# nizepart/Research-and-Development-of-Kubernetes-Operator-for-Machine-Learning-Pipelines

Hardware: AMD Instinct MI355X
Metric: served_tokens_per_sec (higher is better)
Workload: dtype bf16

## Files before the change

research-and-development-of-kubernetes-operator-for-machine-learning-pipelines_amd/ops/__init__.py:

```python
from __future__ import annotations

import math
import os
from pathlib import Path

import torch

from . import reference as ref

_LIB = Path(__file__).resolve().parent / "_C.so"
_loaded = False


class StaleExtension(RuntimeError):
    pass


def load(build_if_missing: bool = True) -> bool:
    global _loaded
    if _loaded:
        return True
    from .build import source_hash

    want = source_hash()
# ... 143 lines not shown


def paged_attention(q, k_cache, v_cache, meta, out: torch.Tensor | None = None,
                    k_scale: torch.Tensor | None = None, v_scale: torch.Tensor | None = None):
    fp8 = _fp8_scales(k_cache, k_scale, v_scale)
    if not q.is_cuda:
        return ref.paged_attention(q, k_cache, v_cache, meta, k_scale, v_scale)
    _need_gpu()
    out = torch.empty_like(q) if out is None else out
    scale = 1.0 / math.sqrt(q.shape[-1])
    window = getattr(meta, "window", 0)
    if fp8:
        pts = getattr(meta, "ptile_seq", None)
        if window or (pts is not None and pts.numel()):
            raise NotImplementedError("fp8 KV cache: no sliding-window and no flash-prefill kernel "
                                      "(build the metadata with flash_min_q = 1 << 30)")
        if meta.tile_seq.numel():
            sem = getattr(meta, "part_sem", None)
            torch.ops.mlop.paged_attention_fp8(out, meta.part_o, meta.part_ml, _no_sem(q.device) if sem is None else sem,
                                               q, k_cache, v_cache, k_scale, v_scale, meta.block_tables,
                                               meta.tile_seq, meta.tile_q0, meta.q_start, meta.q_len, meta.ctx_len,
                                               scale, meta.part_tokens, meta.nparts)
        return out
    if meta.tile_seq.numel():
        sem = getattr(meta, "part_sem", None)
        if sem is None:
            sem = _no_sem(q.device)
        torch.ops.mlop.paged_attention(out, meta.part_o, meta.part_ml, sem, q, k_cache, v_cache,
                                       meta.block_tables, meta.tile_seq, meta.tile_q0, meta.q_start,
                                       meta.q_len, meta.ctx_len, scale, meta.part_tokens, meta.nparts,
                                       window)
    pts = getattr(meta, "ptile_seq", None)
    if pts is not None and pts.numel():
        torch.ops.mlop.flash_prefill(out, q, k_cache, v_cache, meta.block_tables, pts, meta.ptile_q0,
                                     meta.q_start, meta.q_len, meta.ctx_len, scale, window)
    return out


EPI_NONE, EPI_SILU_MUL = 0, 1


def gemm(x: torch.Tensor, w: torch.Tensor, out: torch.Tensor | None = None, epi: int = EPI_NONE):
    N = w.shape[0]
    out_n = N if epi == EPI_NONE else N // 2
    if not x.is_cuda:
        y = torch.nn.functional.linear(x, w) if x.dtype != torch.bfloat16 else \
            torch.nn.functional.linear(x.float(), w.float()).to(x.dtype)
        if epi == EPI_SILU_MUL:
            y = ref.silu_mul(deinterleave_cols(y))
        if out is not None:
            out.copy_(y.view_as(out))
            return out
        return y
    _need_gpu()
    lead = x.shape[:-1]
# ... 646 lines not shown
```

research-and-development-of-kubernetes-operator-for-machine-learning-pipelines_amd/ops/csrc/attention.hip:

```cpp
#include <type_traits>
#include <algorithm>

#include "common.h"
#include "launch.h"

namespace mlop {

__device__ __forceinline__ float fast_exp2(float x) { return __builtin_amdgcn_exp2f(x); }

constexpr int kD = 128;
constexpr int kBS = 16;
constexpr float kNegBig = -1.0e30f;

__device__ __forceinline__ int vswz(int t) { return ((t & 3) << 2) | ((t >> 2) & 3); }
typedef short v4s16 __attribute__((ext_vector_type(4)));
typedef __attribute__((address_space(3))) v4s16 lds_v4s16;

__device__ __forceinline__ uint32_t vt_base(int lane) {
  const int g4 = lane >> 4, q = (lane >> 2) & 3, p = lane & 3;
  const int row = 8 * g4 + q, sw = vswz(row & 15);
  return 256u * row + 16u * ((p >> 1) ^ (sw & 1)) + 8u * (p & 1) + 32u * (sw >> 1);
}
__device__ __forceinline__ bf16x8 vt_frag(uint32_t b, int d) {
  const uint32_t a0 = b ^ (32u * d), a1 = (a0 ^ 16u) + 1024u;
  const v4s16 lo = __builtin_amdgcn_ds_read_tr16_b64_v4i16((lds_v4s16*)(uintptr_t)a0);
  const v4s16 hi = __builtin_amdgcn_ds_read_tr16_b64_v4i16((lds_v4s16*)(uintptr_t)a1);
  bf16x8 f;
#pragma unroll
  for (int e = 0; e < 4; ++e) {
    f[e] = lo[e];
    f[4 + e] = hi[e];
  }
  return f;
}

__device__ __forceinline__ int wid_of(unsigned t) { return __builtin_amdgcn_readfirstlane((int)(t >> 6)); }

__device__ __forceinline__ int window_kv_lo(int p0, int window) { return max(0, p0 - window + 1) & ~31; }


struct KvBf16 {
  const uint16_t* kc;
  const uint16_t* vc;
  static constexpr bool kScaled = false;
  struct Pair {};
  static __device__ __forceinline__ int q_dim(int kk, int g4) { return kk * 32 + g4 * 8; }
  template <int NT>
  __device__ __forceinline__ void load_k(Pair&, int pgA, int pgB, size_t page_stride, int kvh, int lane,
                                         bf16x8 (&ka)[4], bf16x8 (&kb)[4]) const {
    const int r = lane & 15, g4 = lane >> 4;
    const uint16_t* kA = kc + pgA * page_stride + (size_t)kvh * kBS * kD;
    const uint16_t* kB = kc + pgB * page_stride + (size_t)kvh * kBS * kD;
    const uint16_t* kR = (r >> 3 ? kB : kA) + (8 * ((r >> 2) & 1) + (r & 3)) * kD;
#pragma unroll
    for (int kk = 0; kk < 4; ++kk) {
      if constexpr ((NT & 1) != 0) {
        ka[kk] = __builtin_nontemporal_load(reinterpret_cast<const bf16x8*>(kR + kk * 32 + g4 * 8));
        kb[kk] = __builtin_nontemporal_load(reinterpret_cast<const bf16x8*>(kR + 4 * kD + kk * 32 + g4 * 8));
      } else {
        ka[kk] = *reinterpret_cast<const bf16x8*>(kR + kk * 32 + g4 * 8);
        kb[kk] = *reinterpret_cast<const bf16x8*>(kR + 4 * kD + kk * 32 + g4 * 8);
      }
    }
  }
  template <int NT>
  __device__ __forceinline__ void issue_v(Pair&, int pgA, int pgB, size_t page_stride, int kvh, int lane,
                                          uint32_t vimg) const {
    const int r = lane & 15, g4 = lane >> 4;
    asm volatile("s_waitcnt lgkmcnt(0)" ::: "memory");
    const uint16_t* vA = vc + pgA * page_stride + (size_t)kvh * kBS * kD;
    const uint16_t* vB = vc + pgB * page_stride + (size_t)kvh * kBS * kD;
#pragma unroll
    for (int i = 0; i < 8; ++i) {
      const int trow = (4 * i + g4) & 15;
      const uint16_t* src = (i < 4 ? vA : vB) + trow * kD + ((r ^ vswz(trow)) << 3);
      __builtin_amdgcn_global_load_lds((const void*)src, (lds_void_t*)(uintptr_t)(vimg + 1024u * i), 16, 0,
                                       (NT & 1) ? 2  : 0);
    }
  }
  __device__ __forceinline__ void v_ready(const Pair&, int, uint32_t) const {
    asm volatile("s_waitcnt vmcnt(0)" ::: "memory");
  }
  __device__ __forceinline__ void v_read_done() const {}
};

typedef __attribute__((address_space(3))) u32x4 lds_u32x4;

__device__ __forceinline__ bf16x8 cvt8(uint32_t w0, uint32_t w1) {
  const auto f0 = __builtin_amdgcn_cvt_pk_f32_fp8((int)w0, false);
  const auto f1 = __builtin_amdgcn_cvt_pk_f32_fp8((int)w0, true);
  const auto f2 = __builtin_amdgcn_cvt_pk_f32_fp8((int)w1, false);
  const auto f3 = __builtin_amdgcn_cvt_pk_f32_fp8((int)w1, true);
  u32x4 o;
  o[0] = __builtin_amdgcn_perm(__float_as_uint(f0[1]), __float_as_uint(f0[0]), 0x07060302u);
  o[1] = __builtin_amdgcn_perm(__float_as_uint(f1[1]), __float_as_uint(f1[0]), 0x07060302u);
  o[2] = __builtin_amdgcn_perm(__float_as_uint(f2[1]), __float_as_uint(f2[0]), 0x07060302u);
  o[3] = __builtin_amdgcn_perm(__float_as_uint(f3[1]), __float_as_uint(f3[0]), 0x07060302u);
  return __builtin_bit_cast(bf16x8, o);
// ... 1 lines not shown

__device__ __forceinline__ float scale_of(uint32_t w, int i) {
  return __uint_as_float(((w >> (8 * i)) & 0xffu) << 23);
}

template <bool NT>
__device__ __forceinline__ u32x4 load16(const uint8_t* p) {
  if constexpr (NT) return __builtin_nontemporal_load(reinterpret_cast<const u32x4*>(p));
  else return *reinterpret_cast<const u32x4*>(p);
}

struct KvFp8 {
  const uint8_t* kc;
  const uint8_t* vc;
  const uint8_t* ksc;
  const uint8_t* vsc;
  int srow_stride;
  static constexpr bool kScaled = true;
  struct Pair {
    u32x2 ksw, vsw;
    u32x4 vr[4];
  };
  static __device__ __forceinline__ int q_dim(int kk, int g4) { return 64 * (kk >> 1) + 16 * g4 + 8 * (kk & 1); }
  template <int NT>
  __device__ __forceinline__ void load_k(Pair& pr, int pgA, int pgB, size_t page_stride, int kvh, int lane,
                                         bf16x8 (&ka)[4], bf16x8 (&kb)[4]) const {
    const int r = lane & 15, g4 = lane >> 4;
    const uint8_t* kA = kc + pgA * page_stride + (size_t)kvh * kBS * kD;
    const uint8_t* kB = kc + pgB * page_stride + (size_t)kvh * kBS * kD;
    const uint8_t* kR = (r >> 3 ? kB : kA) + (8 * ((r >> 2) & 1) + (r & 3)) * kD + 16 * g4;
    const u32x4 ka0 = load16<(NT & 1) != 0>(kR), ka1 = load16<(NT & 1) != 0>(kR + 64);
    const u32x4 kb0 = load16<(NT & 1) != 0>(kR + 4 * kD), kb1 = load16<(NT & 1) != 0>(kR + 4 * kD + 64);
    const size_t srow = (size_t)(g4 >> 1 ? pgB : pgA) * srow_stride + (size_t)kvh * kBS + 8 * (g4 & 1);
    pr.ksw = *reinterpret_cast<const u32x2*>(ksc + srow);
    pr.vsw = *reinterpret_cast<const u32x2*>(vsc + srow);
    ka[0] = cvt8(ka0[0], ka0[1]); ka[1] = cvt8(ka0[2], ka0[3]);
    ka[2] = cvt8(ka1[0], ka1[1]); ka[3] = cvt8(ka1[2], ka1[3]);
    kb[0] = cvt8(kb0[0], kb0[1]); kb[1] = cvt8(kb0[2], kb0[3]);
    kb[2] = cvt8(kb1[0], kb1[1]); kb[3] = cvt8(kb1[2], kb1[3]);
  }
  template <int NT>
  __device__ __forceinline__ void issue_v(Pair& pr, int pgA, int pgB, size_t page_stride, int kvh, int lane,
                                          uint32_t) const {
    const int v_row = lane >> 3, v_c8 = lane & 7;
    const uint8_t* vA = vc + pgA * page_stride + (size_t)kvh * kBS * kD + v_row * kD + 16 * v_c8;
    const uint8_t* vB = vc + pgB * page_stride + (size_t)kvh * kBS * kD + v_row * kD + 16 * v_c8;
    pr.vr[0] = load16<(NT & 1) != 0>(vA);
    pr.vr[1] = load16<(NT & 1) != 0>(vA + 8 * kD);
    pr.vr[2] = load16<(NT & 1) != 0>(vB);
    pr.vr[3] = load16<(NT & 1) != 0>(vB + 8 * kD);
  }
  __device__ __forceinline__ void v_ready(const Pair& pr, int lane, uint32_t vimg) const {
    const int v_row = lane >> 3, v_c8 = lane & 7;
    const uint32_t v_dst = vimg + 256u * v_row;
#pragma unroll
    for (int j = 0; j < 4; ++j) {
      const int sw = vswz((8 * j + v_row) & 15);
      const uint32_t a = v_dst + 2048u * j;
      *(lds_u32x4*)(uintptr_t)(a + 16u * ((2 * v_c8) ^ sw)) = __builtin_bit_cast(u32x4, cvt8(pr.vr[j][0], pr.vr[j][1]));
      *(lds_u32x4*)(uintptr_t)(a + 16u * ((2 * v_c8 + 1) ^ sw)) = __builtin_bit_cast(u32x4, cvt8(pr.vr[j][2], pr.vr[j][3]));
    }
    asm volatile("" ::: "memory");
  }
  __device__ __forceinline__ void v_read_done() const { asm volatile("" ::: "memory"); }
  static __device__ __forceinline__ float k_scale(const Pair& pr, int h, int i) { return scale_of(pr.ksw[h], i); }
// ... 1 lines not shown
};

__device__ __forceinline__ void combine_slabs(uint16_t* dst, const float* part_o, const float* part_ml,
                                              size_t base, int nvalid, int rr, int c) {
  float M = kNegBig;
  for (int p = 0; p < nvalid; ++p) M = fmaxf(M, part_ml[((base + p) * 16 + rr) * 2]);
  float L = 0.f, acc[8] = {0.f, 0.f, 0.f, 0.f, 0.f, 0.f, 0.f, 0.f};
  for (int p = 0; p < nvalid; ++p) {
    const size_t pb = (base + p) * 16 + rr;
    const float f = exp2f(part_ml[pb * 2] - M);
    L += f * part_ml[pb * 2 + 1];
    const float4* po = reinterpret_cast<const float4*>(part_o + pb * kD + c);
    const float4 x0 = po[0], x1 = po[1];
    acc[0] += f * x0.x; acc[1] += f * x0.y; acc[2] += f * x0.z; acc[3] += f * x0.w;
    acc[4] += f * x1.x; acc[5] += f * x1.y; acc[6] += f * x1.z; acc[7] += f * x1.w;
  }
  const float inv = L > 0.f ? 1.f / L : 0.f;
  u32x4 ov;
#pragma unroll
  for (int j = 0; j < 4; ++j) ov[j] = pack2(acc[2 * j] * inv, acc[2 * j + 1] * inv);
  *reinterpret_cast<u32x4*>(dst) = ov;
}

template <int G, int NT, bool WIN, class KV>
__global__ void __launch_bounds__(256) paged_attn_kernel(
    uint16_t* __restrict__ out, float* __restrict__ part_o, float* __restrict__ part_ml,
    const uint16_t* __restrict__ q, const KV kv, const int* __restrict__ block_tables, int bt_stride,
    const int* __restrict__ tile_seq, const int* __restrict__ tile_q0,
    const int* __restrict__ q_start, const int* __restrict__ q_len,
    const int* __restrict__ ctx_len, int Hq, int Hkv, float scale_log2, int part_tokens,
    int nparts, int num_blocks, int* __restrict__ sem, int window) {
  constexpr int QT = 16 / G;
  __shared__ __attribute__((aligned(256))) float sm_o[4][16][kD + 4];
  __shared__ float sm_m[4][16];
  __shared__ float sm_l[4][16];
  __shared__ int sm_last;

  const int tile = blockIdx.x, kvh = blockIdx.y, part = blockIdx.z;
  const int lane = threadIdx.x & 63, wid = threadIdx.x >> 6;
  const int s = tile_seq[tile], q0 = tile_q0[tile];
  const int* bt = block_tables + (size_t)s * bt_stride;
  int p_begin = part * part_tokens, kv_lo = 0;
  int ql, ctx, qs;
  if constexpr (WIN) {
    ql = q_len[s], ctx = ctx_len[s], qs = q_start[s];
    kv_lo = window_kv_lo(ctx - ql + q0, window);
    p_begin += kv_lo;
  }
  const int bt0 = 2 * ((p_begin >> 5) + wid_of(threadIdx.x));
  const int rawA = bt[min(bt0, bt_stride - 1)], rawB = bt[min(bt0 + 1, bt_stride - 1)];
  if constexpr (!WIN) ql = q_len[s], ctx = ctx_len[s], qs = q_start[s];
  const int last_q = min(q0 + QT, ql) - 1;
  const int kv_end = last_q >= 0 ? ctx - ql + last_q + 1 : 0;
  const int p_end = min(kv_end, p_begin + part_tokens);
  if (p_begin >= p_end && nparts > 1) {
    if (sem != nullptr && part == 0 && kv_end <= 0) {
      const int rr = threadIdx.x >> 4, c = (threadIdx.x & 15) * 8;
      const int qi2 = q0 + rr / G;
      if (qi2 < ql)
        *reinterpret_cast<u32x4*>(out + ((size_t)(qs + qi2) * Hq + kvh * G + (rr % G)) * kD + c) =
            u32x4{0u, 0u, 0u, 0u};
// ... 18 lines not shown
  }

  f32x4 o[8];
#pragma unroll
  for (int d = 0; d < 8; ++d) o[d] = f32x4{0.f, 0.f, 0.f, 0.f};
  float m = kNegBig, l = 0.f;

  const int pp_begin = p_begin >> 5;
  const int pp_end = (p_end + 31) >> 5;
  const int n_pages = (p_end + kBS - 1) / kBS;
  const size_t page_stride = (size_t)Hkv * kBS * kD;

  const uint32_t vimg = (uint32_t)(uintptr_t)&sm_o[0][0][0] + wid * 8448u;
  auto page_a = [&](int pp) { return min(max(bt[2 * pp], 0), num_blocks - 1); };
  auto page_b = [&](int pp, int pa) { return (2 * pp + 1 < n_pages) ? min(max(bt[2 * pp + 1], 0), num_blocks - 1) : pa; };
  int pgA = 0, pgB = 0;
  if (pp_begin + wid < pp_end) {
    pgA = min(max(rawA, 0), num_blocks - 1);
    pgB = (bt0 + 1 < n_pages) ? min(max(rawB, 0), num_blocks - 1) : pgA;
  }
  for (int pp = pp_begin + wid; pp < pp_end; pp += 4) {
    typename KV::Pair pr;
    bf16x8 ka[4], kb[4];
    kv.template load_k<NT>(pr, pgA, pgB, page_stride, kvh, lane, ka, kb);
    kv.template issue_v<NT>(pr, pgA, pgB, page_stride, kvh, lane, vimg);
    if (pp + 4 < pp_end) {
      pgA = page_a(pp + 4);
      pgB = page_b(pp + 4, pgA);
    }
    bf16x8 vf8[8];
    f32x4 sa = {0.f, 0.f, 0.f, 0.f}, sb = {0.f, 0.f, 0.f, 0.f};
#pragma unroll
    for (int kk = 0; kk < 4; ++kk) {
      sa = mfma16(ka[kk], qf[kk], sa);
      sb = mfma16(kb[kk], qf[kk], sb);
    }
    auto s_of = [&](const f32x4& s, int h, int i) {
      if constexpr (KV::kScaled) return s[i] * KV::k_scale(pr, h, i);
      else return s[i];
    };
    const int tokA = pp * 32 + g4 * 8, tokB = tokA + 4;
    float pa[4], pb[4];
    float mx = kNegBig;
#pragma unroll
    for (int i = 0; i < 4; ++i) {
      const int ta = tokA + i, tb = tokB + i;
      if constexpr (WIN) {
        pa[i] = (ta < p_end && ta <= pos_r && ta > pos_r - window) ? s_of(sa, 0, i) * scale_log2 : -INFINITY;
// ... 83 lines not shown
    const size_t slab = (((size_t)tile * Hkv + kvh) * nparts + part) * 16;
    const auto rs_o = __builtin_amdgcn_make_buffer_rsrc(part_o + slab * kD, 0, 16 * kD * 4, 0x00020000);
    const uint32_t oo = (uint32_t)(rr * kD + c) * 4u;
    u32x4 w0, w1;
    w0[0] = __float_as_uint(acc[0]); w0[1] = __float_as_uint(acc[1]);
    w0[2] = __float_as_uint(acc[2]); w0[3] = __float_as_uint(acc[3]);
    w1[0] = __float_as_uint(acc[4]); w1[1] = __float_as_uint(acc[5]);
    w1[2] = __float_as_uint(acc[6]); w1[3] = __float_as_uint(acc[7]);
    __builtin_amdgcn_raw_buffer_store_b128(w0, rs_o, oo, 0, 16 );
    __builtin_amdgcn_raw_buffer_store_b128(w1, rs_o, oo + 16u, 0, 16 );
    if ((threadIdx.x & 15) == 0) {
      const auto rs_ml = __builtin_amdgcn_make_buffer_rsrc(part_ml + slab * 2, 0, 16 * 2 * 4, 0x00020000);
      __builtin_amdgcn_raw_buffer_store_b32(__float_as_uint(M), rs_ml, (uint32_t)rr * 8u, 0, 16);
      __builtin_amdgcn_raw_buffer_store_b32(__float_as_uint(L), rs_ml, (uint32_t)rr * 8u + 4u, 0, 16);
    }
  }
  if (sem == nullptr) return;
  const int nvalid = min(nparts, (kv_end - kv_lo + part_tokens - 1) / part_tokens);
  int* cnt = sem + (size_t)tile * Hkv + kvh;
  asm volatile("s_waitcnt vmcnt(0)" ::: "memory");
  __syncthreads();
  if (threadIdx.x == 0) {
    const int t = __hip_atomic_fetch_add(cnt, 1, __ATOMIC_RELAXED, __HIP_MEMORY_SCOPE_AGENT);
    sm_last = (t == nvalid - 1);
  }
  __syncthreads();
  if (!sm_last) return;
  if (threadIdx.x == 0) {
    __builtin_amdgcn_fence(__ATOMIC_ACQUIRE, "agent");
    asm volatile("s_waitcnt vmcnt(0)" ::: "memory");
    __hip_atomic_store(cnt, 0, __ATOMIC_RELAXED, __HIP_MEMORY_SCOPE_AGENT);
  }
  __syncthreads();
  if (!row_valid) return;
  combine_slabs(out + ((size_t)(qs + qi2) * Hq + head2) * kD + c, part_o, part_ml,
                ((size_t)tile * Hkv + kvh) * nparts, nvalid, rr, c);
}

template <int G, bool WIN = false>
__global__ void __launch_bounds__(256) attn_reduce_kernel(
    uint16_t* __restrict__ out, const float* __restrict__ part_o,
    const float* __restrict__ part_ml, const int* __restrict__ tile_seq,
    const int* __restrict__ tile_q0, const int* __restrict__ q_start,
    const int* __restrict__ q_len, const int* __restrict__ ctx_len, int Hq, int Hkv,
    int part_tokens, int nparts, int window) {
  constexpr int QT = 16 / G;
  const int tile = blockIdx.x, kvh = blockIdx.y;
  const int s = tile_seq[tile], q0 = tile_q0[tile];
  const int ql = q_len[s], ctx = ctx_len[s], qs = q_start[s];
  const int last_q = min(q0 + QT, ql) - 1;
  const int kv_end = last_q >= 0 ? ctx - ql + last_q + 1 : 0;
  const int kv_lo = WIN ? window_kv_lo(ctx - ql + q0, window) : 0;
  const int nvalid = min(nparts, (kv_end - kv_lo + part_tokens - 1) / part_tokens);
  const int rr = threadIdx.x >> 4, c = (threadIdx.x & 15) * 8;
  const int qi = q0 + rr / G;
  if (qi >= ql) return;
  const int head = kvh * G + (rr % G);
  combine_slabs(out + ((size_t)(qs + qi) * Hq + head) * kD + c, part_o, part_ml,
                ((size_t)tile * Hkv + kvh) * nparts, nvalid, rr, c);
// ... 610 lines not shown
__global__ void __launch_bounds__(256, WPC) flash32_prefill_kernel(
    uint16_t* __restrict__ out, const uint16_t* __restrict__ q, const uint16_t* __restrict__ kc,
    const uint16_t* __restrict__ vc, const int* __restrict__ block_tables, int bt_stride,
    const int* __restrict__ ptile_seq, const int* __restrict__ ptile_q0,
    const int* __restrict__ q_start, const int* __restrict__ q_len,
    const int* __restrict__ ctx_len, int Hq, int Hkv, float scale_log2, int num_blocks, int num_ptiles,
    int window) {
  static_assert(!(PERSIST && WIN), "the windowed kernel runs the plain grid only");
  constexpr int STAGES = 3;
  constexpr int STAGE = 4 * kBS * kD;
  __shared__ __attribute__((aligned(256))) uint16_t smem[STAGES * STAGE];
  if constexpr (!PERSIST) {
    flash32_item<G, WIN>(smem, blockIdx.x / Hkv, blockIdx.x % Hkv, out, q, kc, vc, block_tables, bt_stride,
                         ptile_seq, ptile_q0, q_start, q_len, ctx_len, Hq, Hkv, scale_log2, num_blocks, window);
  } else {
    const int kvh = blockIdx.x % Hkv, j = blockIdx.x / Hkv, S = gridDim.x / Hkv;
    for (int r = 0; r * S < num_ptiles; ++r) {
      const int t = r * S + ((r & 1) ? S - 1 - j : j);
      if (t >= num_ptiles) continue;
      if (r > 0) __syncthreads();
      flash32_item<G>(smem, t, kvh, out, q, kc, vc, block_tables, bt_stride, ptile_seq, ptile_q0, q_start, q_len,
                      ctx_len, Hq, Hkv, scale_log2, num_blocks);
    }
  }
}

static int g_flash_persist = 0;
int flash_persist(int set) {
  if (set >= 0) g_flash_persist = set;
  return g_flash_persist;
}

static int g_flash_stream = 0;
int flash_stream(int set) {
  if (set >= 0) g_flash_stream = set;
  return g_flash_stream;
}

static int device_cus() {
  static int cus[16] = {};
  int dev = 0;
  (void)hipGetDevice(&dev);
  if (dev < 0 || dev >= 16) return 256;
  if (cus[dev] == 0) (void)hipDeviceGetAttribute(&cus[dev], hipDeviceAttributeMultiprocessorCount, dev);
  return cus[dev] > 0 ? cus[dev] : 256;
}
// ... 18 lines not shown
    else if (stream)                                                                                     \
      flash32_stream_kernel<GG><<<grid, 256, 0, st>>>(                                                   \
          (uint16_t*)out, (const uint16_t*)q, (const uint16_t*)kc, (const uint16_t*)vc, bt, bt_stride,   \
          ptile_seq, ptile_q0, q_start, q_len, ctx_len, Hq, Hkv, scale_log2, num_blocks, num_ptiles);    \
    else if (persist)                                                                                    \
      flash32_prefill_kernel<GG, 2, true><<<grid, 256, 0, st>>>(                                         \
          (uint16_t*)out, (const uint16_t*)q, (const uint16_t*)kc, (const uint16_t*)vc, bt, bt_stride,   \
          ptile_seq, ptile_q0, q_start, q_len, ctx_len, Hq, Hkv, scale_log2, num_blocks, num_ptiles, 0); \
    else                                                                                                 \
      flash32_prefill_kernel<GG, 2, false><<<grid, 256, 0, st>>>(                                        \
          (uint16_t*)out, (const uint16_t*)q, (const uint16_t*)kc, (const uint16_t*)vc, bt, bt_stride,   \
          ptile_seq, ptile_q0, q_start, q_len, ctx_len, Hq, Hkv, scale_log2, num_blocks, num_ptiles, 0); \
    break;
  switch (Hq / Hkv) {
    MLOP_FLASH_CASE(1)
    MLOP_FLASH_CASE(2)
    MLOP_FLASH_CASE(4)
    MLOP_FLASH_CASE(8)
    default: break;
  }
#undef MLOP_FLASH_CASE
}

}
```

research-and-development-of-kubernetes-operator-for-machine-learning-pipelines_amd/ops/csrc/bindings.cpp:

```cpp
#include <climits>
#include <cstdlib>
#include <string>
#include <torch/library.h>
#include <ATen/ATen.h>
#include <c10/hip/HIPStream.h>
#include <c10/core/DeviceGuard.h>
#include <cmath>

#include "launch.h"
#include "gemm_plan.h"

namespace {

using at::Tensor;

hipStream_t cur_stream() { return c10::hip::getCurrentHIPStream().stream(); }

void check_bf16(const Tensor& t, const char* name) {
  TORCH_CHECK(t.is_cuda(), name, " must be a GPU tensor");
  TORCH_CHECK(t.scalar_type() == at::kBFloat16, name, " must be bf16");
  TORCH_CHECK(t.is_contiguous(), name, " must be contiguous");
}
void check_i32(const Tensor& t, const char* name) {
  TORCH_CHECK(t.is_cuda(), name, " must be a GPU tensor");
// ... 200 lines not shown
  return a;
}

void paged_attention(Tensor out, Tensor part_o, Tensor part_ml, Tensor part_sem, Tensor q, Tensor k_cache,
                     Tensor v_cache, Tensor block_tables, Tensor tile_seq, Tensor tile_q0,
                     Tensor q_start, Tensor q_len, Tensor ctx_len, double scale,
                     int64_t part_tokens, int64_t nparts, int64_t window) {
  TORCH_CHECK(window >= 0 && window < (1 << 30), "window must be >= 0 (0: no sliding window)");
  check_bf16(k_cache, "k_cache"); check_bf16(v_cache, "v_cache");
  TORCH_CHECK(k_cache.dim() == 4 && k_cache.size(2) == 16 && k_cache.size(3) == 128,
              "k_cache must be [NB, Hkv, 16, 128]");
  TORCH_CHECK(v_cache.sizes() == at::IntArrayRef({k_cache.size(0), k_cache.size(1), 16, 128}),
              "v_cache must be [NB, Hkv, 16, 128] (token-major, as k_cache)");
  const DecodeAttention a = check_decode_attention(out, part_o, part_ml, part_sem, q, k_cache, block_tables, tile_seq,
                                                   tile_q0, q_start, q_len, ctx_len, part_tokens, nparts);
  c10::DeviceGuard g(q.device());
  const float scale_log2 = (float)(scale * 1.4426950408889634);
  mlop::launch_paged_attention(
      out.data_ptr(), a.part_o, a.part_ml, q.data_ptr(), k_cache.data_ptr(), v_cache.data_ptr(),
      block_tables.data_ptr<int>(), (int)block_tables.stride(0), tile_seq.data_ptr<int>(),
      tile_q0.data_ptr<int>(), q_start.data_ptr<int>(), q_len.data_ptr<int>(), ctx_len.data_ptr<int>(),
      a.num_tiles, a.Hq, a.Hkv, scale_log2, (int)part_tokens, (int)nparts, (int)k_cache.size(0), a.sem,
      (int)window, cur_stream());
}

void check_fp8_cache(const Tensor& c, const Tensor& sc, const char* name) {
  TORCH_CHECK(c.is_cuda() && c.scalar_type() == at::kFloat8_e4m3fn && c.is_contiguous(), name,
              " must be a contiguous float8_e4m3fn GPU tensor");
  TORCH_CHECK(c.dim() == 4 && c.size(2) == 16 && c.size(3) == 128, name, " must be [NB, Hkv, 16, 128]");
  TORCH_CHECK(sc.is_cuda() && sc.scalar_type() == at::kByte && sc.is_contiguous(), name,
              " scales must be a contiguous uint8 GPU tensor");
  TORCH_CHECK(sc.sizes() == at::IntArrayRef({c.size(0), c.size(1), 16}), name, " scales must be [NB, Hkv, 16]");
  TORCH_CHECK((reinterpret_cast<uintptr_t>(c.data_ptr()) & 15) == 0 &&
                  (reinterpret_cast<uintptr_t>(sc.data_ptr()) & 15) == 0,
              name, " and its scales must be 16-B aligned");
}

void rope_cache_fp8(Tensor q_out, Tensor k_cache, Tensor v_cache, Tensor k_scale, Tensor v_scale, Tensor qkv,
                    Tensor pos, Tensor cos_sin, Tensor slots) {
  check_bf16(q_out, "q_out");
  check_fp8_cache(k_cache, k_scale, "k_cache"); check_fp8_cache(v_cache, v_scale, "v_cache");
  check_i32(pos, "pos"); check_i32(slots, "slots");
  TORCH_CHECK(qkv.is_cuda() && qkv.scalar_type() == at::kBFloat16 && qkv.stride(-1) == 1 && qkv.dim() == 2,
              "qkv must be 2-d bf16 with unit inner stride");
  TORCH_CHECK(cos_sin.is_cuda() && cos_sin.scalar_type() == at::kFloat && cos_sin.is_contiguous(), "cos_sin f32");
  TORCH_CHECK(q_out.dim() == 3 && q_out.size(2) == 128, "q_out must be [T, Hq, 128]");
// ... 763 lines not shown
  m.def("ep_ipc_handle(int h) -> Tensor", &ep_ipc_handle);
  m.def("ep_open(int h, Tensor handles) -> ()", &ep_open);
  m.def("ep_dispatch(int h, Tensor(a!) xp, Tensor(b!) offsets, Tensor x, Tensor topi) -> ()");
  m.def("ep_combine(int h, Tensor(a!) out, Tensor y, Tensor topw, Tensor topi) -> ()");
  m.def("ep_error(int h) -> int", &ep_error);
  m.def("ep_mem_mode(int h) -> int", &ep_mem_mode);
  m.def("ep_destroy(int h) -> ()", &ep_destroy);
  m.def("gemm_workspace(int M, int N, int K, int epi) -> int", &gemm_workspace);
  m.def("gemm_big_variant(int set=-1) -> int", &knob<mlop::gemm_big_variant>);
  m.def("gemm_half_tile(int set=-1) -> int", &knob<mlop::gemm_half_tile>);
  m.def("gemm_small_nt(int set=-1) -> int", &knob<mlop::gemm_small_nt>);
  m.def("attn_kv_nt(int set=-1) -> int", &knob<mlop::attn_kv_nt>);
  m.def("gemm_slab_nt(int set=-1) -> int", &knob<mlop::gemm_slab_nt>);
  m.def("gemm_rope_split(int set=-1) -> int", &knob<mlop::gemm_rope_split>);
  m.def("gemm_split_target(int set=-1) -> int", &knob<mlop::gemm_split_target>);
  m.def("gemm_grouped_narrow(int set=-1) -> int", &knob<mlop::gemm_grouped_narrow>);
  m.def("gemm_ws_max_m(int set=-1) -> int", &knob<mlop::gemm_ws_max_m>);
  m.def("decode_chain_max_m() -> int", &decode_chain_max_m);
  m.def("gemm_ws_plan(int rb, int u, int nt) -> ()", &gemm_ws_plan);
  m.def("gemm_ws_small_m(int set=-1) -> int", &knob<mlop::gemm_ws_small_m>);
  m.def("gemm_ws_rope_m(int set=-1) -> int", &knob<mlop::gemm_ws_rope_m>);
  m.def("flash_persist(int set=-1) -> int", &knob<mlop::flash_persist>);
  m.def("flash_stream(int set=-1) -> int", &knob<mlop::flash_stream>);
  m.def("gemm_grouped_balance(int set=-1) -> int", &knob<mlop::gemm_grouped_balance>);
  m.def("gemm_grouped_order(int set=-1) -> int", &knob<mlop::gemm_grouped_order>);
  m.def("moe_mid_tok(int set=-1) -> int", &knob<mlop::moe_mid_tok>);
  m.def("gemm_mid_chain(int set=-1) -> int", &knob<mlop::gemm_mid_chain>);
  m.def("mid_chain_ok(int M, int N, int K, int epi) -> bool", &mid_chain_ok);
  m.def("moe_mid_max_tokens(int set=-1) -> int", &knob<mlop::moe_mid_max_tokens>);
  m.def("gemm_grouped_plan(int bm, int bn, int stages, int splits) -> ()", &gemm_grouped_plan);
  m.def("gemm_dense_plan(int variant, int bm, int bn, int splits, int stages=0) -> ()", &gemm_dense_plan);
  m.def("gemm_small_stages(int set=-1) -> int", &knob<mlop::gemm_small_stages>);
  m.def("gemm_small_tile(int set=-1) -> int", &knob<mlop::gemm_small_tile>);
  m.def("gemm_sk_mode(int set=-1) -> int", &knob<mlop::gemm_sk_mode>);
  m.def("gemm_sk_reserve() -> bool", &gemm_sk_reserve);
  m.def("gemm_sk_workgroups(int M, int N, int K) -> int", &gemm_sk_workgroups);
  m.def("vmm_supported(int device) -> bool", &vmm_supported);
  m.def("vmm_granularity(int device) -> int", &vmm_granularity);
  m.def("vmm_arena(int bytes, int device) -> Tensor", &vmm_arena);
  m.def("vmm_map_chunks(Tensor flat, int region_stride, int n_regions, int chunk_bytes, int first, "
        "int count, bool async_) -> bool", &vmm_map_chunks);
  m.def("vmm_chunks_ready(Tensor flat) -> int", &vmm_chunks_ready);
  m.def("vmm_error(Tensor flat) -> int", &vmm_error);
  m.def("gemm_rope_supported(int M, int N, int K) -> bool", &gemm_rope_supported);
  m.def("w4_chain_ok(int M, int N, int K) -> bool", &w4_chain_ok);
  m.def("chain_ok(int M, int N, int K, int epi) -> bool", &chain_ok);
// ... 33 lines not shown
  m.def("penalty_update(Tensor(a!) table, int vocab, Tensor slots, Tensor tokens) -> ()");
  m.def("grammar_mask(Tensor(a!) logits, Tensor arena, Tensor base, Tensor rows, Tensor state) -> ()");
  m.def("grammar_advance(Tensor arena, int vocab, Tensor base, Tensor rows, Tensor(a!) state, Tensor tokens) -> ()");
  m.def("apply_penalties(Tensor(a!) logits, Tensor table, Tensor slots, Tensor rep, Tensor freq, "
        "Tensor pres) -> ()");
  m.def("token_logprobs(Tensor(a!) out_lp, Tensor(b!) out_id, Tensor logits, Tensor chosen, Tensor want) -> ()");
  m.def("spec_accept(Tensor sampled, Tensor q_start, Tensor drafts, Tensor nd, Tensor rows, Tensor(a!) hist, "
        "Tensor(b!) hist_len, Tensor(c!) out) -> ()");
  m.def("spec_propose(Tensor hist, Tensor hist_len, Tensor rows, Tensor cap, int n_max, int n_min, "
        "Tensor(a!) out) -> ()");
  m.def("rmsnorm(Tensor(a!) out, Tensor x, Tensor w, float eps) -> ()");
  m.def("add_rmsnorm(Tensor(a!) out, Tensor(b!) residual, Tensor x, Tensor w, float eps) -> ()");
  m.def("rope_cache(Tensor(a!) q_out, Tensor(b!) k_cache, Tensor(c!) v_cache, Tensor qkv, "
        "Tensor pos, Tensor cos_sin, Tensor slots) -> ()");
  m.def("silu_mul(Tensor(a!) out, Tensor x, int interleaved=0) -> ()");
  m.def("lora_shrink(Tensor(a!) tmp, Tensor x, Tensor A, Tensor tok_slot, Tensor slot_rank, int R=16) -> ()");
  m.def("lora_expand_add(Tensor(a!) y, Tensor tmp, Tensor B, Tensor tile_group, Tensor tok_slot, "
        "Tensor slot_rank) -> ()");
  m.def("embedding(Tensor(a!) out, Tensor table, Tensor ids, int vocab_start) -> ()");
  m.def("gemm_ws(Tensor(a!) out, Tensor a, Tensor w, int epi, bool rs, float eps) -> bool");
  m.def("flash_prefill(Tensor(a!) out, Tensor q, Tensor k_cache, Tensor v_cache, Tensor block_tables, "
        "Tensor ptile_seq, Tensor ptile_q0, Tensor q_start, Tensor q_len, Tensor ctx_len, float scale, "
        "int window=0) -> ()");
  m.def("paged_attention(Tensor(a!) out, Tensor(b!) part_o, Tensor(c!) part_ml, Tensor(d!) part_sem, Tensor q, "
        "Tensor k_cache, Tensor v_cache, Tensor block_tables, Tensor tile_seq, Tensor tile_q0, "
        "Tensor q_start, Tensor q_len, Tensor ctx_len, float scale, int part_tokens, "
        "int nparts, int window=0) -> ()");
  m.def("rope_cache_fp8(Tensor(a!) q_out, Tensor(b!) k_cache, Tensor(c!) v_cache, Tensor(d!) k_scale, "
        "Tensor(e!) v_scale, Tensor qkv, Tensor pos, Tensor cos_sin, Tensor slots) -> ()");
  m.def("paged_attention_fp8(Tensor(a!) out, Tensor(b!) part_o, Tensor(c!) part_ml, Tensor(d!) part_sem, Tensor q, "
        "Tensor k_cache, Tensor v_cache, Tensor k_scale, Tensor v_scale, Tensor block_tables, Tensor tile_seq, "
        "Tensor tile_q0, Tensor q_start, Tensor q_len, Tensor ctx_len, float scale, int part_tokens, "
        "int nparts) -> ()");
}

TORCH_LIBRARY_IMPL(mlop, CUDA, m) {
  m.impl("rmsnorm", &rmsnorm);
  m.impl("add_rmsnorm", &add_rmsnorm);
  m.impl("rope_cache", &rope_cache);
  m.impl("silu_mul", &silu_mul);
  m.impl("embedding", &embedding);
  m.impl("lora_shrink", &lora_shrink);
  m.impl("lora_expand_add", &lora_expand_add);
  m.impl("paged_attention", &paged_attention);
  m.impl("rope_cache_fp8", &rope_cache_fp8);
  m.impl("paged_attention_fp8", &paged_attention_fp8);
  m.impl("flash_prefill", &flash_prefill);
  m.impl("gemm", &gemm);
  m.impl("gemm_ws", &gemm_ws);
  m.impl("grouped_gemm", &grouped_gemm);
  m.impl("gemm_add_rmsnorm", &gemm_add_rmsnorm);
  m.impl("gemm_res_ss", &gemm_res_ss);
  m.impl("gemm_rs", &gemm_rs);
  m.impl("gemm_rs_rope", &gemm_rs_rope);
  m.impl("gemm_rope_cache", &gemm_rope_cache);
  m.impl("moe_route", &moe_route);
  m.impl("moe_dispatch_small", &moe_dispatch_small);
  m.impl("moe_dispatch_mid", &moe_dispatch_mid);
  m.impl("moe_down_combine_add_rmsnorm", &moe_down_combine_add_rmsnorm);
  m.impl("moe_combine_add_rmsnorm", &moe_combine_add_rmsnorm);
  m.impl("moe_permute", &moe_permute);
  m.impl("moe_combine", &moe_combine);
  m.impl("argmax", &argmax);
  m.impl("sample", &sample);
  m.impl("penalty_reset", &penalty_reset);
  m.impl("penalty_update", &penalty_update);
  m.impl("grammar_mask", &grammar_mask);
  m.impl("grammar_advance", &grammar_advance);
  m.impl("apply_penalties", &apply_penalties);
  m.impl("token_logprobs", &token_logprobs);
// ... 10 lines not shown
```

research-and-development-of-kubernetes-operator-for-machine-learning-pipelines_amd/ops/csrc/launch.h:

```cpp
#pragma once

#include <string>
#include <hip/hip_runtime.h>
#include <stdint.h>
#include <algorithm>
#include <memory>

namespace mlop {

void launch_rmsnorm(void* out, const void* x, const void* w, float eps, int M, int H,
                    hipStream_t st);
void launch_add_rmsnorm(void* out, void* residual, const void* x, const void* w, float eps, int M,
                        int H, hipStream_t st);
void launch_rope_cache(void* q_out, void* k_cache, void* v_cache, const void* qkv, const int* pos,
                       const float* cos_sin, const int* slots, int T, int Hq, int Hkv, int D,
                       int qkv_stride, int BS, hipStream_t st);
void launch_silu_mul(void* out, const void* x, int M, int I, int interleaved, hipStream_t st);
void launch_device_delay(long long ticks, hipStream_t st);
void launch_lora_shrink(const void* x, int ldx, const void* A, float* tmp, const int* tok_slot,
                        const int* slot_rank, int T, int K, int GR, int R, int S, hipStream_t st);
void launch_lora_expand_add(void* y, int ldy, const float* tmp, const void* B, const uint8_t* tile_group,
                            const int* tok_slot, const int* slot_rank, int T, int N, int GR, int R, int S,
                            hipStream_t st);
void launch_embedding(void* out, const void* table, const long* ids, int T, int H, long vocab_start,
// ... 2 lines not shown
                            const void* kc, const void* vc, const int* bt, int bt_stride,
                            const int* tile_seq, const int* tile_q0, const int* q_start,
                            const int* q_len, const int* ctx_len, int num_tiles, int Hq, int Hkv,
                            float scale_log2, int part_tokens, int nparts, int num_blocks,
                            int* sem, int window, hipStream_t st);
void launch_rope_cache_fp8(void* q_out, void* k_cache, void* v_cache, void* k_scale, void* v_scale,
                           const void* qkv, const int* pos, const float* cos_sin, const int* slots, int T,
                           int Hq, int Hkv, int qkv_stride, int BS, hipStream_t st);
void launch_paged_attention_fp8(void* out, float* part_o, float* part_ml, const void* q, const void* kc,
                                const void* vc, const void* ks, const void* vs, const int* bt,
                                int bt_stride, const int* tile_seq, const int* tile_q0, const int* q_start,
                                const int* q_len, const int* ctx_len, int num_tiles, int Hq, int Hkv,
                                float scale_log2, int part_tokens, int nparts, int num_blocks, int* sem,
                                hipStream_t st);
int flash_persist(int set);
int flash_stream(int set);
int gemm_grouped_balance(int set);
int gemm_grouped_order(int set);
int moe_mid_tok(int set);
void launch_flash_prefill(void* out, const void* q, const void* kc, const void* vc, const int* bt,
                          int bt_stride, const int* ptile_seq, const int* ptile_q0,
                          const int* q_start, const int* q_len, const int* ctx_len, int num_ptiles,
                          int Hq, int Hkv, float scale_log2, int num_blocks, int window, hipStream_t st);
struct RopeEpi {
  uint16_t* q_out;
  uint16_t* k_cache;
  uint16_t* v_cache;
  const int* pos;
  const float* cos_sin;
  const int* slots;
  int Hq, Hkv, BS;
  const float* ss_in = nullptr;
  float* ss_out = nullptr;
  float* ss_tot = nullptr;
  int* ss_cnt = nullptr;
  float ss_inv_k = 0.f, ss_eps = 0.f;
  const int* a_rows = nullptr;
  int b_nt = 0;
  int ws_nt = 0;
  int mid_acq = 0;
};
void launch_rope_cache_slabs(const RopeEpi& re, const float* ws, int splits, int T, int N, hipStream_t st);
bool gemm_sk_scratch(float** ws, int** cnt, int* cus);
bool gemm_sk_available(int* cus);
bool run_w4(int epi, const uint16_t* A, int lda, const uint16_t* B, int ldb, uint16_t* C, int ldc, int M, int N,
            int K, hipStream_t st, const RopeEpi& re, int bm = 256);
// ... 130 lines not shown
```

Measured before the change: 37560.

## Fuse decode and flash-prefill attention into one mixed-batch kernel launch

Adds a mixed attention kernel that runs decode tiles and flash-prefill tiles in a single grid, interleaving flash blocks among decode blocks through a stride map, with one shared LDS arena. It is used when a batch has both kinds of tiles, no sliding window and one partition. This removes the second launch and lets the two workloads fill the GPU together. The bf16 decode path now clamps tail K/V row loads to the valid context, and paged_attn_kernel raises its bf16 occupancy hint to 3 blocks per CU, which may cost register spills.

```diff
diff --git a/research-and-development-of-kubernetes-operator-for-machine-learning-pipelines_amd/ops/__init__.py b/research-and-development-of-kubernetes-operator-for-machine-learning-pipelines_amd/ops/__init__.py
--- a/research-and-development-of-kubernetes-operator-for-machine-learning-pipelines_amd/ops/__init__.py
+++ b/research-and-development-of-kubernetes-operator-for-machine-learning-pipelines_amd/ops/__init__.py
@@ -189,6 +189,13 @@
                                                meta.tile_seq, meta.tile_q0, meta.q_start, meta.q_len, meta.ctx_len,
                                                scale, meta.part_tokens, meta.nparts)
         return out
+    pts = getattr(meta, "ptile_seq", None)
+    if (meta.tile_seq.numel() and pts is not None and pts.numel() and not window and meta.nparts == 1
+            and q.shape[1] // k_cache.shape[1] <= 8 and torch.ops.mlop.attn_mixed_launch(-1)):
+        torch.ops.mlop.mixed_attention(out, q, k_cache, v_cache, meta.block_tables, meta.tile_seq, meta.tile_q0,
+                                       pts, meta.ptile_q0, meta.q_start, meta.q_len, meta.ctx_len, scale,
+                                       meta.part_tokens)
+        return out
     if meta.tile_seq.numel():
         sem = getattr(meta, "part_sem", None)
         if sem is None:
@@ -197,7 +204,6 @@
                                        meta.block_tables, meta.tile_seq, meta.tile_q0, meta.q_start,
                                        meta.q_len, meta.ctx_len, scale, meta.part_tokens, meta.nparts,
                                        window)
-    pts = getattr(meta, "ptile_seq", None)
     if pts is not None and pts.numel():
         torch.ops.mlop.flash_prefill(out, q, k_cache, v_cache, meta.block_tables, pts, meta.ptile_q0,
                                      meta.q_start, meta.q_len, meta.ctx_len, scale, window)
diff --git a/research-and-development-of-kubernetes-operator-for-machine-learning-pipelines_amd/ops/csrc/attention.hip b/research-and-development-of-kubernetes-operator-for-machine-learning-pipelines_amd/ops/csrc/attention.hip
--- a/research-and-development-of-kubernetes-operator-for-machine-learning-pipelines_amd/ops/csrc/attention.hip
+++ b/research-and-development-of-kubernetes-operator-for-machine-learning-pipelines_amd/ops/csrc/attention.hip
@@ -45,26 +45,37 @@
   static constexpr bool kScaled = false;
   struct Pair {};
   static __device__ __forceinline__ int q_dim(int kk, int g4) { return kk * 32 + g4 * 8; }
-  template <int NT>
-  __device__ __forceinline__ void load_k(Pair&, int pgA, int pgB, size_t page_stride, int kvh, int lane,
+  static constexpr bool kClampsTail = true;
+  static __device__ __forceinline__ int last_row(int rem, bool page_b) {
+    return (page_b && rem > kBS ? rem - kBS : min(rem, kBS)) - 1;
+  }
+  template <int NT, bool TAIL>
+  __device__ __forceinline__ void load_k(Pair&, int pgA, int pgB, size_t page_stride, int kvh, int lane, int rem,
                                          bf16x8 (&ka)[4], bf16x8 (&kb)[4]) const {
     const int r = lane & 15, g4 = lane >> 4;
     const uint16_t* kA = kc + pgA * page_stride + (size_t)kvh * kBS * kD;
     const uint16_t* kB = kc + pgB * page_stride + (size_t)kvh * kBS * kD;
-    const uint16_t* kR = (r >> 3 ? kB : kA) + (8 * ((r >> 2) & 1) + (r & 3)) * kD;
+    const int row = 8 * ((r >> 2) & 1) + (r & 3);
+    const uint16_t* kR = (r >> 3 ? kB : kA) + row * kD;
+    int d4 = 4 * kD;
+    if constexpr (TAIL) {
+      const int last = last_row(rem, r >> 3), ra = min(row, last);
+      kR += (ra - row) * kD;
+      d4 = (min(row + 4, last) - ra) * kD;
+    }
 #pragma unroll
     for (int kk = 0; kk < 4; ++kk) {
       if constexpr ((NT & 1) != 0) {
         ka[kk] = __builtin_nontemporal_load(reinterpret_cast<const bf16x8*>(kR + kk * 32 + g4 * 8));
-        kb[kk] = __builtin_nontemporal_load(reinterpret_cast<const bf16x8*>(kR + 4 * kD + kk * 32 + g4 * 8));
+        kb[kk] = __builtin_nontemporal_load(reinterpret_cast<const bf16x8*>(kR + d4 + kk * 32 + g4 * 8));
       } else {
         ka[kk] = *reinterpret_cast<const bf16x8*>(kR + kk * 32 + g4 * 8);
-        kb[kk] = *reinterpret_cast<const bf16x8*>(kR + 4 * kD + kk * 32 + g4 * 8);
-      }
-    }
-  }
-  template <int NT>
-  __device__ __forceinline__ void issue_v(Pair&, int pgA, int pgB, size_t page_stride, int kvh, int lane,
+        kb[kk] = *reinterpret_cast<const bf16x8*>(kR + d4 + kk * 32 + g4 * 8);
+      }
+    }
+  }
+  template <int NT, bool TAIL>
+  __device__ __forceinline__ void issue_v(Pair&, int pgA, int pgB, size_t page_stride, int kvh, int lane, int rem,
                                           uint32_t vimg) const {
     const int r = lane & 15, g4 = lane >> 4;
     asm volatile("s_waitcnt lgkmcnt(0)" ::: "memory");
@@ -73,7 +84,8 @@
 #pragma unroll
     for (int i = 0; i < 8; ++i) {
       const int trow = (4 * i + g4) & 15;
-      const uint16_t* src = (i < 4 ? vA : vB) + trow * kD + ((r ^ vswz(trow)) << 3);
+      const int srow = TAIL ? min(trow, last_row(rem, i >= 4)) : trow;
+      const uint16_t* src = (i < 4 ? vA : vB) + srow * kD + ((r ^ vswz(trow)) << 3);
       __builtin_amdgcn_global_load_lds((const void*)src, (lds_void_t*)(uintptr_t)(vimg + 1024u * i), 16, 0,
                                        (NT & 1) ? 2  : 0);
     }
@@ -121,8 +133,9 @@
     u32x4 vr[4];
   };
   static __device__ __forceinline__ int q_dim(int kk, int g4) { return 64 * (kk >> 1) + 16 * g4 + 8 * (kk & 1); }
-  template <int NT>
-  __device__ __forceinline__ void load_k(Pair& pr, int pgA, int pgB, size_t page_stride, int kvh, int lane,
+  static constexpr bool kClampsTail = false;
+  template <int NT, bool TAIL>
+  __device__ __forceinline__ void load_k(Pair& pr, int pgA, int pgB, size_t page_stride, int kvh, int lane, int,
                                          bf16x8 (&ka)[4], bf16x8 (&kb)[4]) const {
     const int r = lane & 15, g4 = lane >> 4;
     const uint8_t* kA = kc + pgA * page_stride + (size_t)kvh * kBS * kD;
@@ -138,8 +151,8 @@
     kb[0] = cvt8(kb0[0], kb0[1]); kb[1] = cvt8(kb0[2], kb0[3]);
     kb[2] = cvt8(kb1[0], kb1[1]); kb[3] = cvt8(kb1[2], kb1[3]);
   }
-  template <int NT>
-  __device__ __forceinline__ void issue_v(Pair& pr, int pgA, int pgB, size_t page_stride, int kvh, int lane,
+  template <int NT, bool TAIL>
+  __device__ __forceinline__ void issue_v(Pair& pr, int pgA, int pgB, size_t page_stride, int kvh, int lane, int,
                                           uint32_t) const {
     const int v_row = lane >> 3, v_c8 = lane & 7;
     const uint8_t* vA = vc + pgA * page_stride + (size_t)kvh * kBS * kD + v_row * kD + 16 * v_c8;
@@ -187,21 +200,17 @@
   *reinterpret_cast<u32x4*>(dst) = ov;
 }
 
+constexpr int kDecodeLdsO = 4 * 16 * (kD + 4) * 4, kDecodeLdsM = 4 * 16 * 4;
 template <int G, int NT, bool WIN, class KV>
-__global__ void __launch_bounds__(256) paged_attn_kernel(
+__device__ __forceinline__ void decode_tile(
+    float (*sm_o)[16][kD + 4], float (*sm_m)[16], float (*sm_l)[16], int* sm_last, int tile, int kvh, int part,
     uint16_t* __restrict__ out, float* __restrict__ part_o, float* __restrict__ part_ml,
-    const uint16_t* __restrict__ q, const KV kv, const int* __restrict__ block_tables, int bt_stride,
+    const uint16_t* __restrict__ q, const KV& kv, const int* __restrict__ block_tables, int bt_stride,
     const int* __restrict__ tile_seq, const int* __restrict__ tile_q0,
     const int* __restrict__ q_start, const int* __restrict__ q_len,
     const int* __restrict__ ctx_len, int Hq, int Hkv, float scale_log2, int part_tokens,
     int nparts, int num_blocks, int* __restrict__ sem, int window) {
   constexpr int QT = 16 / G;
-  __shared__ __attribute__((aligned(256))) float sm_o[4][16][kD + 4];
-  __shared__ float sm_m[4][16];
-  __shared__ float sm_l[4][16];
-  __shared__ int sm_last;
-
-  const int tile = blockIdx.x, kvh = blockIdx.y, part = blockIdx.z;
   const int lane = threadIdx.x & 63, wid = threadIdx.x >> 6;
   const int s = tile_seq[tile], q0 = tile_q0[tile];
   const int* bt = block_tables + (size_t)s * bt_stride;
@@ -266,8 +275,14 @@
   for (int pp = pp_begin + wid; pp < pp_end; pp += 4) {
     typename KV::Pair pr;
     bf16x8 ka[4], kb[4];
-    kv.template load_k<NT>(pr, pgA, pgB, page_stride, kvh, lane, ka, kb);
-    kv.template issue_v<NT>(pr, pgA, pgB, page_stride, kvh, lane, vimg);
+    const int rem = p_end - pp * 32;
+    if (!KV::kClampsTail || rem >= 32) {
+      kv.template load_k<NT, false>(pr, pgA, pgB, page_stride, kvh, lane, rem, ka, kb);
+      kv.template issue_v<NT, false>(pr, pgA, pgB, page_stride, kvh, lane, rem, vimg);
+    } else {
+      kv.template load_k<NT, true>(pr, pgA, pgB, page_stride, kvh, lane, rem, ka, kb);
+      kv.template issue_v<NT, true>(pr, pgA, pgB, page_stride, kvh, lane, rem, vimg);
+    }
     if (pp + 4 < pp_end) {
       pgA = page_a(pp + 4);
       pgB = page_b(pp + 4, pgA);
@@ -397,10 +412,10 @@
   __syncthreads();
   if (threadIdx.x == 0) {
     const int t = __hip_atomic_fetch_add(cnt, 1, __ATOMIC_RELAXED, __HIP_MEMORY_SCOPE_AGENT);
-    sm_last = (t == nvalid - 1);
+    *sm_last = (t == nvalid - 1);
   }
   __syncthreads();
-  if (!sm_last) return;
+  if (!*sm_last) return;
   if (threadIdx.x == 0) {
     __builtin_amdgcn_fence(__ATOMIC_ACQUIRE, "agent");
     asm volatile("s_waitcnt vmcnt(0)" ::: "memory");
@@ -410,6 +425,23 @@
   if (!row_valid) return;
   combine_slabs(out + ((size_t)(qs + qi2) * Hq + head2) * kD + c, part_o, part_ml,
                 ((size_t)tile * Hkv + kvh) * nparts, nvalid, rr, c);
+}
+
+template <int G, int NT, bool WIN, class KV>
+__global__ void __launch_bounds__(256, KV::kClampsTail ? 3 : 1) paged_attn_kernel(
+    uint16_t* __restrict__ out, float* __restrict__ part_o, float* __restrict__ part_ml,
+    const uint16_t* __restrict__ q, const KV kv, const int* __restrict__ block_tables, int bt_stride,
+    const int* __restrict__ tile_seq, const int* __restrict__ tile_q0,
+    const int* __restrict__ q_start, const int* __restrict__ q_len,
+    const int* __restrict__ ctx_len, int Hq, int Hkv, float scale_log2, int part_tokens,
+    int nparts, int num_blocks, int* __restrict__ sem, int window) {
+  __shared__ __attribute__((aligned(256))) float sm_o[4][16][kD + 4];
+  __shared__ float sm_m[4][16];
+  __shared__ float sm_l[4][16];
+  __shared__ int sm_last;
+  decode_tile<G, NT, WIN, KV>(sm_o, sm_m, sm_l, &sm_last, blockIdx.x, blockIdx.y, blockIdx.z, out, part_o, part_ml,
+                              q, kv, block_tables, bt_stride, tile_seq, tile_q0, q_start, q_len, ctx_len, Hq, Hkv,
+                              scale_log2, part_tokens, nparts, num_blocks, sem, window);
 }
 
 template <int G, bool WIN = false>
@@ -1066,6 +1098,31 @@
       flash32_item<G>(smem, t, kvh, out, q, kc, vc, block_tables, bt_stride, ptile_seq, ptile_q0, q_start, q_len,
                       ctx_len, Hq, Hkv, scale_log2, num_blocks);
     }
+  }
+}
+
+template <int G, int NT>
+__global__ void __launch_bounds__(256, 3) mixed_attn_kernel(
+    uint16_t* __restrict__ out, const uint16_t* __restrict__ q, const KvBf16 kv,
+    const int* __restrict__ block_tables, int bt_stride, const int* __restrict__ tile_seq,
+    const int* __restrict__ tile_q0, const int* __restrict__ ptile_seq, const int* __restrict__ ptile_q0,
+    const int* __restrict__ q_start, const int* __restrict__ q_len, const int* __restrict__ ctx_len, int Hq,
+    int Hkv, float scale_log2, int part_tokens, int num_blocks, int num_tiles, int n_flash, int stride) {
+  constexpr int kFlashLds = 3 * 4 * kBS * kD * 2;
+  constexpr int kDecodeLds = kDecodeLdsO + 2 * kDecodeLdsM + 4;
+  __shared__ __attribute__((aligned(256))) unsigned char arena[kFlashLds > kDecodeLds ? kFlashLds : kDecodeLds];
+  const MixedItem it = mixed_attn_item(blockIdx.x, n_flash, stride);
+  if (it.flash) {
+    flash32_item<G>(reinterpret_cast<uint16_t*>(arena), it.item / Hkv, it.item % Hkv, out, q, kv.kc, kv.vc,
+                    block_tables, bt_stride, ptile_seq, ptile_q0, q_start, q_len, ctx_len, Hq, Hkv, scale_log2,
+                    num_blocks);
+  } else {
+    decode_tile<G, NT, false, KvBf16>(
+        reinterpret_cast<float(*)[16][kD + 4]>(arena), reinterpret_cast<float(*)[16]>(arena + kDecodeLdsO),
+        reinterpret_cast<float(*)[16]>(arena + kDecodeLdsO + kDecodeLdsM),
+        reinterpret_cast<int*>(arena + kDecodeLdsO + 2 * kDecodeLdsM), it.item % num_tiles, it.item / num_tiles, 0,
+        out, nullptr, nullptr, q, kv, block_tables, bt_stride, tile_seq, tile_q0, q_start, q_len, ctx_len, Hq, Hkv,
+        scale_log2, part_tokens, 1, num_blocks, nullptr, 0);
   }
 }
 
@@ -1130,4 +1187,35 @@
 #undef MLOP_FLASH_CASE
 }
 
-}
+static int g_attn_mixed_launch = 1;
+int attn_mixed_launch(int set) {
+  if (set >= 0) g_attn_mixed_launch = set;
+  return g_attn_mixed_launch;
+}
+
+void launch_mixed_attention(void* out, const void* q, const void* kc, const void* vc, const int* bt,
+                            int bt_stride, const int* tile_seq, const int* tile_q0, const int* ptile_seq,
+                            const int* ptile_q0, const int* q_start, const int* q_len, const int* ctx_len,
+                            int num_tiles, int num_ptiles, int Hq, int Hkv, float scale_log2, int part_tokens,
+                            int num_blocks, hipStream_t st) {
+  const int F = num_ptiles * Hkv, D = num_tiles * Hkv;
+  const int S = mixed_attn_stride(F, D);
+  const int nt = num_tiles >= 8 ? g_attn_kv_nt : 0;
+  const KvBf16 kv{(const uint16_t*)kc, (const uint16_t*)vc};
+  auto go = [&](auto g_tag) {
+    constexpr int G = decltype(g_tag)::value;
+    auto kern = nt == 3 ? mixed_attn_kernel<G, 3> : nt ? mixed_attn_kernel<G, 1> : mixed_attn_kernel<G, 0>;
+    kern<<<dim3(F + D), 256, 0, st>>>((uint16_t*)out, (const uint16_t*)q, kv, bt, bt_stride, tile_seq, tile_q0,
+                                      ptile_seq, ptile_q0, q_start, q_len, ctx_len, Hq, Hkv, scale_log2,
+                                      part_tokens, num_blocks, num_tiles, F, S);
+  };
+  switch (Hq / Hkv) {
+    case 1: go(std::integral_constant<int, 1>{}); break;
+    case 2: go(std::integral_constant<int, 2>{}); break;
+    case 4: go(std::integral_constant<int, 4>{}); break;
+    case 8: go(std::integral_constant<int, 8>{}); break;
+    default: break;
+  }
+}
+
+}
diff --git a/research-and-development-of-kubernetes-operator-for-machine-learning-pipelines_amd/ops/csrc/bindings.cpp b/research-and-development-of-kubernetes-operator-for-machine-learning-pipelines_amd/ops/csrc/bindings.cpp
--- a/research-and-development-of-kubernetes-operator-for-machine-learning-pipelines_amd/ops/csrc/bindings.cpp
+++ b/research-and-development-of-kubernetes-operator-for-machine-learning-pipelines_amd/ops/csrc/bindings.cpp
@@ -246,6 +246,43 @@
       tile_q0.data_ptr<int>(), q_start.data_ptr<int>(), q_len.data_ptr<int>(), ctx_len.data_ptr<int>(),
       a.num_tiles, a.Hq, a.Hkv, scale_log2, (int)part_tokens, (int)nparts, (int)k_cache.size(0), a.sem,
       (int)window, cur_stream());
+}
+
+void mixed_attention(Tensor out, Tensor q, Tensor k_cache, Tensor v_cache, Tensor block_tables, Tensor tile_seq,
+                     Tensor tile_q0, Tensor ptile_seq, Tensor ptile_q0, Tensor q_start, Tensor q_len,
+                     Tensor ctx_len, double scale, int64_t part_tokens) {
+  check_bf16(k_cache, "k_cache"); check_bf16(v_cache, "v_cache");
+  TORCH_CHECK(k_cache.dim() == 4 && k_cache.size(2) == 16 && k_cache.size(3) == 128,
+              "k_cache must be [NB, Hkv, 16, 128]");
+  TORCH_CHECK(v_cache.sizes() == at::IntArrayRef({k_cache.size(0), k_cache.size(1), 16, 128}),
+              "v_cache must be [NB, Hkv, 16, 128] (token-major, as k_cache)");
+  const DecodeAttention a = check_decode_attention(out, out, out, out, q, k_cache, block_tables, tile_seq, tile_q0,
+                                                   q_start, q_len, ctx_len, part_tokens, 1);
+  check_i32(ptile_seq, "ptile_seq"); check_i32(ptile_q0, "ptile_q0");
+  TORCH_CHECK(ptile_seq.numel() == ptile_q0.numel(), "tile arrays");
+  TORCH_CHECK(a.num_tiles > 0 && ptile_seq.numel() > 0, "mixed attention needs decode tiles and flash tiles");
+  TORCH_CHECK(a.Hq / a.Hkv <= 8, "mixed attention: GQA group must be 1, 2, 4 or 8");
+  TORCH_CHECK((ptile_seq.numel() + (int64_t)a.num_tiles) * a.Hkv < (int64_t)0x7fffffff, "mixed attention: grid");
+  c10::DeviceGuard g(q.device());
+  mlop::launch_mixed_attention(
+      out.data_ptr(), q.data_ptr(), k_cache.data_ptr(), v_cache.data_ptr(), block_tables.data_ptr<int>(),
+      (int)block_tables.stride(0), tile_seq.data_ptr<int>(), tile_q0.data_ptr<int>(), ptile_seq.data_ptr<int>(),
+      ptile_q0.data_ptr<int>(), q_start.data_ptr<int>(), q_len.data_ptr<int>(), ctx_len.data_ptr<int>(),
+      a.num_tiles, (int)ptile_seq.numel(), a.Hq, a.Hkv, (float)(scale * 1.4426950408889634), (int)part_tokens,
+      (int)k_cache.size(0), cur_stream());
+}
+
+Tensor mixed_attn_block_map(int64_t F, int64_t D) {
+  TORCH_CHECK(F >= 0 && D >= 0 && F + D < (int64_t)0x7fffffff, "item counts");
+  Tensor map = at::empty({F + D, 2}, at::TensorOptions().dtype(at::kInt));
+  int* p = map.data_ptr<int>();
+  const int S = mlop::mixed_attn_stride((int)F, (int)D);
+  for (int64_t b = 0; b < F + D; ++b) {
+    const mlop::MixedItem it = mlop::mixed_attn_item((int)b, (int)F, S);
+    p[2 * b] = it.flash ? 1 : 0;
+    p[2 * b + 1] = it.item;
+  }
+  return map;
 }
 
 void check_fp8_cache(const Tensor& c, const Tensor& sc, const char* name) {
@@ -1055,6 +1092,8 @@
   m.def("gemm_ws_rope_m(int set=-1) -> int", &knob<mlop::gemm_ws_rope_m>);
   m.def("flash_persist(int set=-1) -> int", &knob<mlop::flash_persist>);
   m.def("flash_stream(int set=-1) -> int", &knob<mlop::flash_stream>);
+  m.def("attn_mixed_launch(int set=-1) -> int", &knob<mlop::attn_mixed_launch>);
+  m.def("mixed_attn_block_map(int F, int D) -> Tensor", &mixed_attn_block_map);
   m.def("gemm_grouped_balance(int set=-1) -> int", &knob<mlop::gemm_grouped_balance>);
   m.def("gemm_grouped_order(int set=-1) -> int", &knob<mlop::gemm_grouped_order>);
   m.def("moe_mid_tok(int set=-1) -> int", &knob<mlop::moe_mid_tok>);
@@ -1134,6 +1173,9 @@
   m.def("flash_prefill(Tensor(a!) out, Tensor q, Tensor k_cache, Tensor v_cache, Tensor block_tables, "
         "Tensor ptile_seq, Tensor ptile_q0, Tensor q_start, Tensor q_len, Tensor ctx_len, float scale, "
         "int window=0) -> ()");
+  m.def("mixed_attention(Tensor(a!) out, Tensor q, Tensor k_cache, Tensor v_cache, Tensor block_tables, "
+        "Tensor tile_seq, Tensor tile_q0, Tensor ptile_seq, Tensor ptile_q0, Tensor q_start, Tensor q_len, "
+        "Tensor ctx_len, float scale, int part_tokens) -> ()");
   m.def("paged_attention(Tensor(a!) out, Tensor(b!) part_o, Tensor(c!) part_ml, Tensor(d!) part_sem, Tensor q, "
         "Tensor k_cache, Tensor v_cache, Tensor block_tables, Tensor tile_seq, Tensor tile_q0, "
         "Tensor q_start, Tensor q_len, Tensor ctx_len, float scale, int part_tokens, "
@@ -1158,6 +1200,7 @@
   m.impl("rope_cache_fp8", &rope_cache_fp8);
   m.impl("paged_attention_fp8", &paged_attention_fp8);
   m.impl("flash_prefill", &flash_prefill);
+  m.impl("mixed_attention", &mixed_attention);
   m.impl("gemm", &gemm);
   m.impl("gemm_ws", &gemm_ws);
   m.impl("grouped_gemm", &grouped_gemm);
diff --git a/research-and-development-of-kubernetes-operator-for-machine-learning-pipelines_amd/ops/csrc/launch.h b/research-and-development-of-kubernetes-operator-for-machine-learning-pipelines_amd/ops/csrc/launch.h
--- a/research-and-development-of-kubernetes-operator-for-machine-learning-pipelines_amd/ops/csrc/launch.h
+++ b/research-and-development-of-kubernetes-operator-for-machine-learning-pipelines_amd/ops/csrc/launch.h
@@ -48,6 +48,26 @@
                           int bt_stride, const int* ptile_seq, const int* ptile_q0,
                           const int* q_start, const int* q_len, const int* ctx_len, int num_ptiles,
                           int Hq, int Hkv, float scale_log2, int num_blocks, int window, hipStream_t st);
+struct MixedItem {
+  bool flash;
+  int item;
+};
+__host__ __device__ inline int mixed_attn_stride(int F, int D) {
+  const long s = F > 0 ? ((long)F + D) / (2L * F) : 1;
+  return s < 1 ? 1 : (int)s;
+}
+__host__ __device__ inline MixedItem mixed_attn_item(int block, int F, int S) {
+  const int k = block / S;
+  if (k < F && block - k * S == 0) return MixedItem{true, k};
+  const int before = (block + S - 1) / S;
+  return MixedItem{false, block - (before < F ? before : F)};
+}
+int attn_mixed_launch(int set);
+void launch_mixed_attention(void* out, const void* q, const void* kc, const void* vc, const int* bt,
+                            int bt_stride, const int* tile_seq, const int* tile_q0, const int* ptile_seq,
+                            const int* ptile_q0, const int* q_start, const int* q_len, const int* ctx_len,
+                            int num_tiles, int num_ptiles, int Hq, int Hkv, float scale_log2, int part_tokens,
+                            int num_blocks, hipStream_t st);
 struct RopeEpi {
   uint16_t* q_out;
   uint16_t* k_cache;
```

Result: no change. 37790 (median of 6 runs) (+0.6%).
